# kvcache-ai/ktransformers

Hardware: NVIDIA H100
Metric: decode tok/s DeepSeek-V3 671B INT4 (Q4_K_M) MoE-block hot path; HBM GB/s vs roofline (higher is better)
Workload: dtype int8xint4/int6->int32 dp4a, fp32 scales+accumulate, bf16 in/out

## Files before the change

ktransformers_b200/csrc/gate.cuh:

```cuda
#pragma once
#include "common.cuh"

namespace ktb {

constexpr int kGateWarps = 4;
constexpr int kGateThreads = kGateWarps * 32;
constexpr int kGateTokTile = 8;

struct GateParams {
    const float* W;
    const void* x;
    int hidden_type, E, H, T, S;
    int top_k, n_group, topk_group, scoring, topk_method, norm_topk_prob;
    float routed_scaling_factor;
    const float* bias;
    float* partial;
    float* logits_out;
    int64_t* idx;
    float* w;
    const int* bsz;
    unsigned* ticket;
};

static inline int gate_splits(int E, int H, int nsms) {
    int S = nsms * 12 / E;
    if (S < 1) S = 1;
    if (S > 8) S = 8;
    while (S > 1 && H / 4 / S < 64) S--;
    return S;
}

constexpr int kGateEPT = 4;

static inline bool gate_config_ok(const ktb200_gate_config* c) {
    if (c->n_experts <= 0 || c->n_experts > kGateThreads * kGateEPT || c->hidden_size <= 0 || c->hidden_size % 4 || c->top_k <= 0 ||
        c->top_k > 32 || c->top_k > c->n_experts) {
        set_error("gate: bad shape (E=%d H=%d top_k=%d; E<=%d, top_k<=32, H%%4==0)", c->n_experts, c->hidden_size, c->top_k,
                  kGateThreads * kGateEPT);
        return false;
    }
    if (c->n_group < 1 || c->n_group > 32 || c->n_experts % c->n_group || c->topk_group < 1 || c->topk_group > c->n_group) {
        set_error("gate: bad grouping (n_group=%d topk_group=%d)", c->n_group, c->topk_group);
        return false;
    }
    if (c->scoring < 0 || c->scoring > 1 || c->topk_method < 0 || c->topk_method > 2) { set_error("gate: bad scoring/topk_method"); return false; }
    const int gs = c->n_experts / c->n_group;
    if (c->topk_method == 0 && c->n_group > 1 && gs < 2) {
        set_error("gate: noaux_tc needs at least 2 experts per group (E=%d n_group=%d)", c->n_experts, c->n_group);
        return false;
    }
    if (c->topk_method != 1 && c->n_group > 1 && c->top_k > c->topk_group * gs) {
        set_error("gate: top_k=%d exceeds the %d experts of topk_group=%d groups", c->top_k, c->topk_group * gs, c->topk_group);
        return false;
    }
    if (!is_hidden_type(c->hidden_type) || !c->weight) { set_error("gate: bad hidden_type or null weight"); return false; }
    return true;
}

__device__ __forceinline__ unsigned fkey(float f) {
    const unsigned u = __float_as_uint(f);
    return (u & 0x80000000u) ? ~u : (u | 0x80000000u);
}

__device__ __forceinline__ float fkey_inv(unsigned k) {
    return __uint_as_float((k & 0x80000000u) ? (k & 0x7fffffffu) : ~k);
}

template <int BAR>
__device__ __forceinline__ void gate_sync() {
    if (BAR == 0) __syncthreads();
    else asm volatile("bar.sync %0, %1;" ::"n"(BAR), "n"(kGateThreads) : "memory");
}
struct GateSel {
    int E, S, top_k, n_group, topk_group, scoring, topk_method, norm_topk_prob;
    float routed_scaling_factor;
    const float* bias;
    const float* partial;
};
template <int BAR>
__device__ void gate_select_token(const GateParams& pin, int t, float* sm, int64_t* idx_out, float* w_out, float* logits_out) {
    const GateSel p{pin.E, pin.S, pin.top_k, pin.n_group, pin.topk_group, pin.scoring, pin.topk_method, pin.norm_topk_prob,
                    pin.routed_scaling_factor, pin.bias, pin.partial};
    const int E = p.E, tid = threadIdx.x, lane = tid & 31, warp = tid >> 5;
    float* scores = sm;
    float* choice = sm + E;
    float* gsc = choice + E;
    unsigned* wbest = reinterpret_cast<unsigned*>(gsc + 32);
    float* red = reinterpret_cast<float*>(wbest + 2 * kGateWarps);

    float v[kGateEPT], pv[8][kGateEPT];
#pragma unroll
    for (int s = 0; s < 8; s++) {
        const float* pp = p.partial + ((long)t * p.S + s) * E;
#pragma unroll
        for (int i = 0; i < kGateEPT; i++) {
            const int e = tid + kGateThreads * i;
            pv[s][i] = (s < p.S && e < E) ? __ldcg(pp + e) : 0.f;
        }
    }
    float bv[kGateEPT];
#pragma unroll
    for (int i = 0; i < kGateEPT; i++) {
        const int e = tid + kGateThreads * i;
        bv[i] = (p.topk_method == 0 && p.bias && e < E) ? __ldg(p.bias + e) : 0.f;
    }
#pragma unroll
    for (int i = 0; i < kGateEPT; i++) {
        v[i] = 0.f;
#pragma unroll
        for (int s = 0; s < 8; s++)
            if (s < p.S) v[i] += pv[s][i];
    }
    if (logits_out) {
#pragma unroll
        for (int i = 0; i < kGateEPT; i++) {
            const int e = tid + kGateThreads * i;
            if (e < E) logits_out[(long)t * E + e] = v[i];
        }
    }
    if (p.scoring == 0) {
#pragma unroll
        for (int i = 0; i < kGateEPT; i++) v[i] = __fdiv_rn(1.0f, 1.0f + expf(-v[i]));
    } else {
        float m = -INFINITY;
#pragma unroll
        for (int i = 0; i < kGateEPT; i++) if (tid + kGateThreads * i < E) m = fmaxf(m, v[i]);
#pragma unroll
        for (int o = 16; o > 0; o >>= 1) m = fmaxf(m, __shfl_xor_sync(0xffffffffu, m, o));
        if (lane == 0) red[warp] = m;
        gate_sync<BAR>();
        m = red[0];
        for (int w = 1; w < kGateWarps; w++) m = fmaxf(m, red[w]);
        float sum = 0.f;
#pragma unroll
        for (int i = 0; i < kGateEPT; i++) {
            v[i] = (tid + kGateThreads * i < E) ? expf(v[i] - m) : 0.f;
            sum += v[i];
        }
        sum = warp_sum(sum);
        if (lane == 0) red[kGateWarps + warp] = sum;
        gate_sync<BAR>();
        sum = 0.f;
        for (int w = 0; w < kGateWarps; w++) sum += red[kGateWarps + w];
#pragma unroll
        for (int i = 0; i < kGateEPT; i++) v[i] = __fdiv_rn(v[i], sum);
    }
    float c[kGateEPT];
#pragma unroll
    for (int i = 0; i < kGateEPT; i++) {
        const int e = tid + kGateThreads * i;
        c[i] = -INFINITY;
        if (e < E) {
            c[i] = v[i] + bv[i];
            scores[e] = v[i];
            choice[e] = c[i];
        }
    }
    gate_sync<BAR>();

    if (p.n_group > 1 && p.topk_method != 1) {
        const int gs = E / p.n_group;
        for (int g = warp; g < p.n_group; g += kGateWarps) {
            float a1 = -INFINITY, a2 = -INFINITY;
            for (int i = lane; i < gs; i += 32) {
                const float x = choice[g * gs + i];
                if (x > a1) { a2 = a1; a1 = x; } else if (x > a2) { a2 = x; }
            }
            const unsigned k1 = fkey(a1);
            const unsigned mx1 = __reduce_max_sync(0xffffffffu, k1);
            const int wl = __ffs(__ballot_sync(0xffffffffu, k1 == mx1)) - 1;
            const unsigned mx2 = __reduce_max_sync(0xffffffffu, lane == wl ? fkey(a2) : k1);
            if (lane == 0) gsc[g] = (p.topk_method == 0) ? (fkey_inv(mx1) + fkey_inv(mx2)) : fkey_inv(mx1);
        }
        gate_sync<BAR>();
        const float fill = (p.topk_method == 0) ? -INFINITY : 0.0f;
#pragma unroll
        for (int i = 0; i < kGateEPT; i++) {
            const int e = tid + kGateThreads * i;
            if (e < E) {
                const int g = e / gs;
                const float mine = gsc[g];
                int rank = 0;
                for (int o = 0; o < p.n_group; o++) {
                    const float og = gsc[o];
                    rank += (og > mine || (og == mine && o < g)) ? 1 : 0;
                }
                if (rank >= p.topk_group) { c[i] = fill; choice[e] = fill; }
            }
        }
        gate_sync<BAR>();
    }

    if (warp == 0) {
        constexpr int EPL = kGateThreads * kGateEPT / 32;
        unsigned ck[EPL];
#pragma unroll
        for (int i = 0; i < EPL; i++) {
            const int e = lane + 32 * i;
            ck[i] = (e < E) ? fkey(choice[e]) : 0u;
        }
        float wsum = 0.f, myw = 0.f;
        long myidx = 0;
        for (int it = 0; it < p.top_k; it++) {
            unsigned bk = 0;
            int bi = 0x7fffffff;
#pragma unroll
            for (int i = 0; i < EPL; i++)
                if (ck[i] > bk) { bk = ck[i]; bi = lane + 32 * i; }
            const unsigned mx = __reduce_max_sync(0xffffffffu, bk);
            int win = __reduce_min_sync(0xffffffffu, (bk == mx) ? bi : 0x7fffffff);
            if (win == 0x7fffffff || win < 0 || win >= E) win = 0;
            const float wv = (p.topk_method == 2) ? choice[win] : scores[win];
#pragma unroll
            for (int i = 0; i < EPL; i++)
                if (lane + 32 * i == win) ck[i] = 0u;
            if (lane == it) { myw = wv; myidx = win; }
            wsum += wv;
        }
        if (lane < p.top_k) {
            float w = myw;
            const bool do_norm = p.top_k > 1 && p.norm_topk_prob;
            if (do_norm) w = __fdiv_rn(w, wsum + 1e-20f);
            if (p.topk_method == 0 || !do_norm) w = w * p.routed_scaling_factor;
            idx_out[lane] = myidx;
            w_out[lane] = w;
        }
    }
    gate_sync<BAR>();
}

template <int NT>
__device__ __forceinline__ void gate_dot(const GateParams& p, const float4* wrow, const float* xs, int nc4, int lane, int t0, int e,
                                         int s, int S, int nt = NT) {
    float acc[NT];
#pragma unroll
    for (int i = 0; i < NT; i++) acc[i] = 0.f;
    for (int cb = lane; cb < nc4; cb += 32 * 8) {
        float4 w[8];
#pragma unroll
        for (int u = 0; u < 8; u++) {
// ... 27 lines not shown
```

ktransformers_b200/csrc/moe_block.cu:

```cuda
#include <cstdlib>

#include "gate.cuh"
#include "gemv_bulk.cuh"
#include "handles.cuh"

namespace ktb {

constexpr int kBlockWarps = 15;
constexpr int kBlockWarpsLo = 12;

struct BlockParams {
    GateParams g;
    const void *w_gate, *w_up, *w_down;
    const void *s_gate, *s_up, *s_down;
    int n_local, id_offset;
    int H, I, k;
    int hidden_type, use_silu;
    float* inter;
    void* out;
    unsigned* sync;
    unsigned* ready;
    unsigned* status;
    uint8_t* stage_q;
    int16_t* stage_bs;
    float* stage_d;
    int nrows_max;
    int region_a;
    int ring_bytes;
    int prime_u, prime_d;
    unsigned long long* trace;
    const uint8_t* pf[3];
    unsigned pf_bytes[3];
};

__device__ __forceinline__ unsigned ld_acquire_u32(const unsigned* p) {
    unsigned v;
    asm volatile("ld.acquire.gpu.global.u32 %0, [%1];" : "=r"(v) : "l"(p) : "memory");
    return v;
}
__device__ __forceinline__ unsigned ld_acquire_sys_u32(const unsigned* p) {
    unsigned v;
    asm volatile("ld.acquire.sys.global.u32 %0, [%1];" : "=r"(v) : "l"(p) : "memory");
    return v;
}
__device__ __forceinline__ unsigned long long ep_now() {
    unsigned long long t;
    asm volatile("mov.u64 %0, %%globaltimer;" : "=l"(t));
    return t;
}
constexpr unsigned long long kEpTimeoutNs = 4000000000ull;
template <bool SYS>
__device__ __forceinline__ void wait_ge(const unsigned* p, unsigned target, unsigned* status) {
    unsigned long long t0 = 0;
    unsigned spins = 0;
    while ((int)((SYS ? ld_acquire_sys_u32(p) : ld_acquire_u32(p)) - target) < 0) {
        if ((++spins & 1023u) == 0) {
            const unsigned long long t = ep_now();
            if (!t0) t0 = t;
            else if (t - t0 > kEpTimeoutNs) { *status = 1; break; }
        }
    }
}

__device__ __forceinline__ void red_release_gpu_add(unsigned* p, unsigned v) {
    asm volatile("red.release.gpu.global.add.u32 [%0], %1;" ::"l"(p), "r"(v) : "memory");
}
__device__ __forceinline__ void grid_arrive(unsigned* counter, unsigned& gen) {
    __syncthreads();
    gen++;
    if (threadIdx.x == 0) red_release_gpu_add(counter, 1u);
}
__device__ __forceinline__ void grid_wait(unsigned* counter, unsigned gen) {
    if (threadIdx.x == 0) {
        const unsigned target = gen * gridDim.x;
        while (ld_acquire_u32(counter) < target) {}
    }
    __syncthreads();
}


__device__ __forceinline__ void trace_stamp(const BlockParams& p, int i) {
    if (p.trace) p.trace[blockIdx.x * 16 + i] = ep_now();
}
__device__ __forceinline__ void block_stamp(const BlockParams& p, int i) {
    if (threadIdx.x == 0) trace_stamp(p, i);
}

__device__ __forceinline__ float4 load_x4(const void* x, long i4, int type) {
    if (type == KTB200_TYPE_F32) return reinterpret_cast<const float4*>(x)[i4];
    const uint2 v = reinterpret_cast<const uint2*>(x)[i4];
    if (type == KTB200_TYPE_BF16)
        return make_float4(__uint_as_float(v.x << 16), __uint_as_float(v.x & 0xffff0000u), __uint_as_float(v.y << 16),
                           __uint_as_float(v.y & 0xffff0000u));
    const float2 a = __half22float2(*reinterpret_cast<const __half2*>(&v.x)), b = __half22float2(*reinterpret_cast<const __half2*>(&v.y));
    return make_float4(a.x, a.y, b.x, b.y);
}

struct BlockShared {
    BlockParams prm;
    int64_t ids[32];
    float w[32];
    int vs[36];
    int nv;
    unsigned skip;
    int ent_state[36];
    int last_cta;
};
constexpr int kBlockSharedBytes = (sizeof(BlockShared) + 15) & ~15;

struct BlockLay {
    uint8_t *xq, *aq;
    int16_t *xbs, *abs_;
    float *xdx, *adx, *sel, *partial;
    size_t ring_off;
};
template <int KBS>
__device__ __forceinline__ BlockLay block_layout(const BlockParams& p, uint8_t* smem) {
    const int nblk = p.H / QK_K, nb = p.I / QK_K, ns = p.k + (p.s_gate ? 1 : 0);
    uint8_t* a = smem + kBlockSharedBytes;
    BlockLay L;
    L.xq = a;
    L.xbs = reinterpret_cast<int16_t*>(a + (size_t)nblk * kActBlkStride);
    L.xdx = reinterpret_cast<float*>(a + (size_t)nblk * (kActBlkStride + 16));
    L.sel = reinterpret_cast<float*>(a + (((size_t)nblk * (kActBlkStride + 16 + 4) + 15) & ~(size_t)15));
    L.aq = a;
    L.abs_ = reinterpret_cast<int16_t*>(a + (size_t)ns * nb * kActBlkStride);
    L.adx = reinterpret_cast<float*>(a + (size_t)ns * nb * (kActBlkStride + 2 * KBS));
    L.partial = reinterpret_cast<float*>(a + p.region_a);
    L.ring_off = ((size_t)kBlockSharedBytes + p.region_a + (size_t)p.nrows_max * ns * 4 + 15) & ~(size_t)15;
    return L;
}

__device__ __forceinline__ void blk_quantize_x(int t) {
    extern __shared__ __align__(16) uint8_t smem[];
    const BlockParams& p = reinterpret_cast<const BlockShared*>(smem)->prm;
    const BlockLay L = block_layout<8>(p, smem);
    const int lane = threadIdx.x & 31, warp = threadIdx.x >> 5, W = blockDim.x >> 5, nblk = p.H / QK_K;
    float cur[8], nxt[8];
    int b = warp;
    if (b < nblk) load_block8(p.g.x, (long)t * p.H + (long)b * QK_K + lane * 8, p.hidden_type, cur);
#pragma unroll 1
    while (b < nblk) {
        const int bn = b + W;
        if (bn < nblk) load_block8(p.g.x, (long)t * p.H + (long)bn * QK_K + lane * 8, p.hidden_type, nxt);
        warp_quantize_q8k_block(cur, lane, reinterpret_cast<uint32_t*>(L.xq + (size_t)b * kActBlkStride), L.xdx + b, nullptr, L.xbs + b * 8);
#pragma unroll
        for (int i = 0; i < 8; i++) cur[i] = nxt[i];
        b = bn;
    }
}

__device__ __forceinline__ void blk_router(int t, bool& waited) {
    extern __shared__ __align__(16) uint8_t smem[];
    const BlockParams& p = reinterpret_cast<const BlockShared*>(smem)->prm;
    const int lane = threadIdx.x & 31, warp = threadIdx.x >> 5, W = blockDim.x >> 5;
    const int E = p.g.E, S = p.g.S, n4 = p.H / 4;
    const int gw = blockIdx.x * W + warp, tw = gridDim.x * W;
    for (int u = gw; u < E * S; u += tw) {
        const int s = u / E, e = u - s * E;
        const int c0 = (int)((long)n4 * s / S), nc4 = (int)((long)n4 * (s + 1) / S) - c0;
        const float4* wrow = reinterpret_cast<const float4*>(p.g.W + (long)e * p.H) + c0;
        const long xbase = (long)t * n4 + c0;
        float acc = 0.f;
        constexpr int NQ = 10;
        for (int cb = lane; cb < nc4; cb += 32 * NQ) {
            float4 w[NQ], xv[NQ];
#pragma unroll
            for (int q = 0; q < NQ; q++) {
                const int c = cb + 32 * q;
// ... 26 lines not shown
    extern __shared__ __align__(16) uint8_t smem[];
    const BlockParams& p = reinterpret_cast<const BlockShared*>(smem)->prm;
    const int lane = threadIdx.x & 31, warp = threadIdx.x >> 5, W = blockDim.x >> 5;
    const int E = p.g.E, S = p.g.S, n4 = p.H / 4, CH = p.ring_bytes / (16 * 32) * 32;
    const int gw = blockIdx.x * W + warp, tw = gridDim.x * W;
    const float4* ring = reinterpret_cast<const float4*>(smem + (ring_u32 - (uint32_t)__cvta_generic_to_shared(smem)));
    auto request = [&](int u, int cs) {
        const int s = u / E, e = u - s * E;
        const int c0 = (int)((long)n4 * s / S), nc4 = (int)((long)n4 * (s + 1) / S) - c0;
        if (lane == 0) {
            const uint32_t bytes = (uint32_t)min(CH, nc4 - cs) * 16u;
            mbar_expect_tx(bar, bytes);
            bulk_g2s(ring_u32, reinterpret_cast<const float4*>(p.g.W + (long)e * p.H) + c0 + cs, bytes, bar);
        }
    };
    if (gw < E * S) request(gw, 0);
    if (!waited) { griddep_wait(); waited = true; }
    blk_quantize_x(t);
    block_stamp(p, 1);
    for (int u = gw; u < E * S; u += tw) {
        const int s = u / E;
        const int c0 = (int)((long)n4 * s / S), nc4 = (int)((long)n4 * (s + 1) / S) - c0;
        const long xbase = (long)t * n4 + c0;
        float acc = 0.f;
        for (int cs = 0; cs < nc4; cs += CH) {
            if (u != gw || cs != 0) request(u, cs);
            const int n = min(CH, nc4 - cs);
            mbar_wait(bar, phase & 1u);
            phase ^= 1u;
            constexpr int NQ = 10;
            for (int cb = lane; cb < n; cb += 32 * NQ) {
                float4 xv[NQ];
#pragma unroll
                for (int q = 0; q < NQ; q++) {
                    const int c = cb + 32 * q;
                    if (c < n) xv[q] = load_x4(p.g.x, xbase + cs + c, p.hidden_type);
                }
#pragma unroll
                for (int q = 0; q < NQ; q++) {
                    const int c = cb + 32 * q;
                    if (c < n) {
                        const float4 w = ring[c];
                        acc = fmaf(w.x, xv[q].x, acc);
                        acc = fmaf(w.y, xv[q].y, acc);
                        acc = fmaf(w.z, xv[q].z, acc);
                        acc = fmaf(w.w, xv[q].w, acc);
                    }
                }
            }
            __syncwarp();
        }
        const float v = warp_sum(acc);
        if (lane == 0) p.g.partial[((long)t * S + s) * E + (u - s * E)] = v;
    }
}

__device__ __forceinline__ void blk_select(int t) {
    extern __shared__ __align__(16) uint8_t smem[];
    BlockShared& sh = *reinterpret_cast<BlockShared*>(smem);
    const BlockParams& p = sh.prm;
    const BlockLay L = block_layout<8>(p, smem);
    const int k = p.k;
    if ((threadIdx.x >> 5) < kGateWarps) {
        gate_select_token<1>(p.g, t, L.sel, sh.ids, sh.w, blockIdx.x == 0 ? p.g.logits_out : nullptr);
    }
    __syncthreads();
    block_stamp(p, 10);
    if (threadIdx.x < 32) {
        const int j = threadIdx.x, e0 = p.s_gate ? 1 : 0;
        const long e = j < k ? (long)sh.ids[j] - p.id_offset : -1;
        const bool own = e >= 0 && e < p.n_local;
        const unsigned m = __ballot_sync(0xffffffffu, own);
        if (own) sh.vs[e0 + __popc(m & ((1u << j) - 1u))] = j;
        if (j == 0) {
            sh.nv = e0 + __popc(m);
            sh.skip = ~m & ((1u << k) - 1u);
        }
    }
    if (blockIdx.x == 0 && threadIdx.x < k) {
        p.g.idx[(long)t * k + threadIdx.x] = sh.ids[threadIdx.x];
        p.g.w[(long)t * k + threadIdx.x] = sh.w[threadIdx.x];
    }
    __syncthreads();
}

__device__ __forceinline__ void entry_slice(int I, int ie, int& r0, int& len) {
    const unsigned s = (blockIdx.x + (unsigned)ie) % gridDim.x;
    r0 = (int)((unsigned long long)I * s / gridDim.x);
    len = (int)((unsigned long long)I * (s + 1) / gridDim.x) - r0;
}

constexpr unsigned kInterEmpty = 0xffffffffu;
__device__ __forceinline__ void st_relaxed_f32(float* p, float v) {
    asm volatile("st.relaxed.gpu.global.f32 [%0], %1;" ::"l"(p), "f"(v) : "memory");
}
__device__ __forceinline__ uint4 ld_relaxed_u4(const void* p) {
    uint4 v;
    asm volatile("ld.relaxed.gpu.global.v4.u32 {%0, %1, %2, %3}, [%4];" : "=r"(v.x), "=r"(v.y), "=r"(v.z), "=r"(v.w) : "l"(p) : "memory");
    return v;
}

template <int KBS>
__device__ __forceinline__ void quantise_block(const BlockParams& p, long gb, float* src) {
    const int lane = threadIdx.x & 31;
    uint4 v0, v1;
    unsigned long long t0 = 0;
    for (unsigned spins = 1;; spins++) {
        v0 = ld_relaxed_u4(src + lane * 8);
        v1 = ld_relaxed_u4(src + lane * 8 + 4);
        const bool here = v0.x != kInterEmpty && v0.y != kInterEmpty && v0.z != kInterEmpty && v0.w != kInterEmpty &&
                          v1.x != kInterEmpty && v1.y != kInterEmpty && v1.z != kInterEmpty && v1.w != kInterEmpty;
        if (__all_sync(0xffffffffu, here)) break;
        if ((spins & 255u) == 0) {
            const unsigned long long t = ep_now();
            if (!t0) t0 = t;
            else if (t - t0 > kEpTimeoutNs) { if (lane == 0) *p.status = 1; break; }
        }
    }
    const float x[8] = {__uint_as_float(v0.x), __uint_as_float(v0.y), __uint_as_float(v0.z), __uint_as_float(v0.w),
                        __uint_as_float(v1.x), __uint_as_float(v1.y), __uint_as_float(v1.z), __uint_as_float(v1.w)};
    warp_quantize_q8k_block(x, lane, reinterpret_cast<uint32_t*>(p.stage_q + gb * QK_K), p.stage_d + gb,
                            KBS == 16 ? p.stage_bs + gb * 16 : nullptr, KBS == 8 ? p.stage_bs + gb * 8 : nullptr);
    const uint4 empty = make_uint4(kInterEmpty, kInterEmpty, kInterEmpty, kInterEmpty);
    reinterpret_cast<uint4*>(src + lane * 8)[0] = empty;
    reinterpret_cast<uint4*>(src + lane * 8)[1] = empty;
    __syncwarp();
    if (lane == 0) {
        __threadfence();
        atomicExch(p.ready + gb, 2u);
    }
}

template <int KBS>
__device__ __forceinline__ void claim_entry(const BlockParams& p, int t, int slot) {
    const int lane = threadIdx.x & 31, ns = p.k + (p.s_gate ? 1 : 0), nb = p.I / QK_K;
    const long g0 = ((long)t * ns + slot) * nb;
    for (int c0 = 0; c0 < nb; c0 += 32) {
        const int nc = min(32, nb - c0), rot = (int)(blockIdx.x % nc);
        for (;;) {
            const unsigned fr = __ballot_sync(0xffffffffu, lane < nc && ld_acquire_u32(p.ready + g0 + c0 + lane) == 0u);
            if (!fr) break;
            const unsigned pref = fr & (~0u << rot);
            const int b = c0 + __ffs(pref ? pref : fr) - 1;
            unsigned won = 0;
            if (lane == 0) won = atomicCAS(p.ready + g0 + b, 0u, 1u) == 0u;
            if (__shfl_sync(0xffffffffu, won, 0)) quantise_block<KBS>(p, g0 + b, p.inter + ((long)t * ns + slot) * p.I + (long)b * QK_K);
        }
    }
}

template <int KBS>
__device__ __forceinline__ void entry_to_smem(BlockShared& sh, const BlockLay& L, int t, int ev, bool need) {
    const BlockParams& p = sh.prm;
    const int lane = threadIdx.x & 31;
    volatile int* state = &sh.ent_state[ev];
    int s = lane == 0 ? *state : 0;
    s = __shfl_sync(0xffffffffu, s, 0);
    if (s == 0) {
        if (lane == 0) s = atomicCAS(&sh.ent_state[ev], 0, 1) == 0 ? 3 : 1;
        s = __shfl_sync(0xffffffffu, s, 0);
    }
    if (s == 3) {
        const int nb = p.I / QK_K, slot = sh.vs[ev];
        const long g0 = ((long)t * (p.k + (p.s_gate ? 1 : 0)) + slot) * nb;
        for (int b = lane; b < nb; b += 32) wait_ge<false>(p.ready + g0 + b, 2u, p.status);
        __syncwarp();
// ... 45 lines not shown
    BlockShared& sh = *reinterpret_cast<BlockShared*>(smem);
    const int lane = threadIdx.x & 31, warp = threadIdx.x >> 5, W = blockDim.x >> 5;
    griddep_launch_dependents();
    bool waited = false;
    int Teff = p.g.T;
    if (p.g.bsz) { griddep_wait(); waited = true; Teff = min(Teff, *p.g.bsz); }
    const int k = p.k;
    const bool has_shared = p.s_gate != nullptr;
    uint32_t bar_u32, ring_u32;
    {
        const BlockLay L = block_layout<DownFmt::kBs>(p, smem);
        const int bar_bytes = (W * SU * 8 + 15) & ~15;
        bar_u32 = (uint32_t)__cvta_generic_to_shared(smem + L.ring_off) + warp * SU * 8;
        ring_u32 = (uint32_t)__cvta_generic_to_shared(smem + L.ring_off + bar_bytes) + warp * p.ring_bytes;
    }
    if (lane == 0) {
#pragma unroll
        for (int s = 0; s < SU; s++) mbar_init(bar_u32 + 8 * s, 1);
        mbar_fence_init();
        fence_proxy_async_smem();
    }
    {
        const uint32_t* src = reinterpret_cast<const uint32_t*>(&p);
        uint32_t* dst = reinterpret_cast<uint32_t*>(&sh.prm);
        for (int i = threadIdx.x; i < (int)(sizeof(BlockParams) / 4); i += blockDim.x) dst[i] = src[i];
    }
    if (threadIdx.x == 0 && has_shared) sh.vs[0] = k;
    uint32_t phase = 0;
    unsigned gen = 0;
    block_stamp(p, 0);

  for (int t = 0; t < Teff; t++) {
    __syncthreads();
    {
        const int nblk = p.H / QK_K, row_bytes = nblk * SZ_Q4_K;
        const int ns = k + (has_shared ? 1 : 0);
        int ie = 0, ir = 0, ir0 = 0, ilen = 0, ileft = 0, isub = 0;
        int ce = 0, cr = 0, cr0 = 0, clen = 0, cleft = 0, csub = 0;
        int stride = W, iend = 1;
        int slot_i = 0, slot_u = 0;
        auto advance = [&](int& e, int& r, int& r0, int& len, int n) {
            int off = r - r0 + n;
            while (off >= len && e + 1 < iend) { off -= len; e++; entry_slice(p.I, e, r0, len); }
            r = r0 + off;
        };
        auto start_list = [&](int e0, int e1, int first, int count, int stride_) {
            iend = e1;
            ie = e0;
            entry_slice(p.I, e0, ir0, ilen);
            ir = ir0;
            advance(ie, ir, ir0, ilen, first);
            ce = ie; cr = ir; cr0 = ir0; clen = ilen;
            ileft = cleft = count > 0 ? count : 0;
            stride = stride_;
        };
        auto issue_u = [&]() {
            if (ileft > 0 && isub - csub < SU) {
                if (lane == 0) {
                    const int s = sh.vs[ie];
                    const bool second = isub & 1;
                    const uint8_t* src;
                    if (s == k) {
                        src = reinterpret_cast<const uint8_t*>(second ? p.s_up : p.s_gate) + (long)ir * row_bytes;
                    } else {
                        const long e = (long)sh.ids[s] - p.id_offset;
                        src = reinterpret_cast<const uint8_t*>(second ? p.w_up : p.w_gate) + (e * p.I + ir) * row_bytes;
                    }
                    const uint32_t bar = bar_u32 + 8 * slot_i;
                    mbar_expect_tx(bar, (uint32_t)row_bytes);
                    bulk_g2s(ring_u32 + slot_i * row_bytes, src, (uint32_t)row_bytes, bar);
                }
                isub++;
                if (!(isub & 1)) {
                    ileft--;
                    advance(ie, ir, ir0, ilen, stride);
                }
                slot_i = (slot_i + 1 == SU) ? 0 : slot_i + 1;
            }
        };
        if (threadIdx.x < 36) sh.ent_state[threadIdx.x] = 0;
        blk_router_ring(t, waited, bar_u32, ring_u32, phase);
        block_stamp(p, 2);
        grid_arrive(p.sync, gen);
        if (has_shared && warp >= kGateWarps) {
            int r0, nr;
            entry_slice(p.I, 0, r0, nr);
            const int first = warp - kGateWarps, st = W - kGateWarps;
            start_list(0, 1, first, (nr - first + st - 1) / st, st);
        }
#pragma unroll
        for (int s = 0; s < SU; s++)
            if (s < p.prime_u) issue_u();
        grid_wait(p.sync, gen);
        block_stamp(p, 3);
        const BlockLay L = block_layout<DownFmt::kBs>(p, smem);
        const uint8_t* ring = smem + (ring_u32 - (uint32_t)__cvta_generic_to_shared(smem));
#pragma unroll 1
        for (int list = 0; list < 2; list++) {
            if (list == 1) {
                blk_select(t);
                block_stamp(p, 4);
                const int e0 = has_shared ? 1 : 0, nv = sh.nv;
                const unsigned G = gridDim.x, s0 = (blockIdx.x + (unsigned)e0) % G;
                auto rows_before = [&](unsigned sl) { return (int)(sl / G) * p.I + (int)((unsigned long long)p.I * (sl % G) / G); };
                const int total = rows_before(s0 + (unsigned)(nv - e0)) - rows_before(s0);
                start_list(e0, nv, warp, (total - warp + W - 1) / W, W);
#pragma unroll
                for (int s = 0; s < SU; s++) issue_u();
            }
            float acc_first = 0.f;
            bool stamp_first = list == 1 && warp == 0;
            while (cleft > 0) {
                mbar_wait(bar_u32 + 8 * slot_u, (phase >> slot_u) & 1u);
                phase ^= 1u << slot_u;
                if (stamp_first) {
                    if (lane == 0) trace_stamp(p, 11);
                    stamp_first = false;
                }
                const uint8_t* row0 = ring + slot_u * row_bytes;
                float acc = 0.f;
                if (lane < nblk)
                    acc = q4k_block_dot(row0 + lane * SZ_Q4_K, L.xq + (size_t)lane * kActBlkStride,
                                        *reinterpret_cast<const uint4*>(L.xbs + lane * 8), L.xdx[lane]);
                __syncwarp();
                slot_u = (slot_u + 1 == SU) ? 0 : slot_u + 1;
                csub++;
                issue_u();
                if (csub & 1) { acc_first = acc; continue; }
                float g = acc_first, uu = acc;
#pragma unroll
                for (int o = 16; o > 0; o >>= 1) {
                    g += __shfl_xor_sync(0xffffffffu, g, o);
                    uu += __shfl_xor_sync(0xffffffffu, uu, o);
                }
                if (lane == 0) st_relaxed_f32(p.inter + ((long)t * ns + sh.vs[ce]) * p.I + cr, (p.use_silu ? act_silu(g) : act_relu(g)) * uu);
                cleft--;
                advance(ce, cr, cr0, clen, stride);
            }
        }
        __syncthreads();
        block_stamp(p, 5);
    }
    {
        const int nb = p.I / QK_K, nrb = RW * nb, item_bytes = nrb * DownFmt::kBlockBytes;
        const int quads = p.H / RW;
        const int q0 = (int)((long)quads * blockIdx.x / gridDim.x), nquads = (int)((long)quads * (blockIdx.x + 1) / gridDim.x) - q0;
        const int nv = sh.nv;
        const int Wd = W - 1;
        int ni = warp < Wd ? nquads * nv - warp : 0;
        ni = ni > 0 ? (ni + Wd - 1) / Wd : 0;
        int dvi = 0, dq = 0, dss = 0, dcons = 0;
        if (ni > 0) { dvi = warp / nquads; dq = warp - dvi * nquads; }
        int evi = dvi, eq = dq;
        int dslot_i = 0, dslot_u = 0;
        auto issue_d = [&]() {
            if (dss < ni && dss - dcons < SD) {
                if (lane == 0) {
                    const int j = sh.vs[dvi];
                    long row = (long)(q0 + dq) * RW;
                    const uint8_t* wbase = reinterpret_cast<const uint8_t*>(p.w_down);
                    if (j == k) wbase = reinterpret_cast<const uint8_t*>(p.s_down);
                    else row += ((long)sh.ids[j] - p.id_offset) * p.H;
                    const uint32_t bar = bar_u32 + 8 * dslot_i;
                    mbar_expect_tx(bar, (uint32_t)item_bytes);
                    bulk_g2s(ring_u32 + dslot_i * item_bytes, wbase + (row >> 2) * item_bytes, (uint32_t)item_bytes, bar);
                }
                dss++;
                dq += Wd;
                while (dq >= nquads) { dq -= nquads; dvi++; }
                dslot_i = (dslot_i + 1 == SD) ? 0 : dslot_i + 1;
            }
        };
#pragma unroll
        for (int s = 0; s < SD; s++) issue_d();
        const BlockLay L = block_layout<DownFmt::kBs>(p, smem);
        if (warp == W - 1) {
            for (int ev = 0; ev < nv; ev++) claim_entry<DownFmt::kBs>(p, t, sh.vs[ev]);
        }
        if (t == Teff - 1 && warp == W - 1) {
#pragma unroll
            for (int r = 0; r < 3; r++) {
                if (p.pf[r]) {
                    const unsigned per = ((p.pf_bytes[r] / gridDim.x) + 15u) & ~15u;
                    const unsigned lo = per * blockIdx.x, hi = min(p.pf_bytes[r], lo + per);
                    for (unsigned o = lo + lane * 4096u; o < hi; o += 32u * 4096u) prefetch_l2_bulk(p.pf[r] + o, min(4096u, hi - o) & ~15u);
                }
            }
        }

        const uint8_t* ring = smem + (ring_u32 - (uint32_t)__cvta_generic_to_shared(smem));
        const int ns = k + (has_shared ? 1 : 0);
        for (int n = 0; n < ni; n++) {
            if (eq < Wd) {
                entry_to_smem<DownFmt::kBs>(sh, L, t, evi, true);
                if (evi + 1 < nv) entry_to_smem<DownFmt::kBs>(sh, L, t, evi + 1, false);
            }
            mbar_wait(bar_u32 + 8 * dslot_u, (phase >> dslot_u) & 1u);
            phase ^= 1u << dslot_u;
            const uint8_t* sl = ring + dslot_u * item_bytes;
            const int j = sh.vs[evi];
            float res;
            {
                float acc[RW] = {0.f, 0.f, 0.f, 0.f};
                for (int f = lane; f < nrb; f += 32) {
                    const int rw = f / nb, blk = f - rw * nb;
                    const int ab = j * nb + blk;
                    const float val = DownFmt::dot(sl, f, nrb, L.aq + (size_t)ab * kActBlkStride, L.abs_ + ab * DownFmt::kBs, L.adx[ab]);
                    acc[0] += rw == 0 ? val : 0.f; acc[1] += rw == 1 ? val : 0.f; acc[2] += rw == 2 ? val : 0.f; acc[3] += rw == 3 ? val : 0.f;
                }
                res = warp_reduce4(acc[0], acc[1], acc[2], acc[3], lane);
            }
            __syncwarp();
            dslot_u = (dslot_u + 1 == SD) ? 0 : dslot_u + 1;
            dcons++;
            issue_d();
            if ((lane & 7) == 0) L.partial[(eq * RW + (lane >> 3)) * ns + j] = res;
            eq += Wd;
            while (eq >= nquads) { eq -= nquads; evi++; }
        }
        __syncthreads();
        block_stamp(p, 8);
        blk_combine<DownFmt::kBs>(t);
        block_stamp(p, 9);
    }
  }

    __syncthreads();
    if (threadIdx.x == 0) sh.last_cta = atomicAdd(p.sync + 1, 1u) == gridDim.x - 1;
    __syncthreads();
    if (sh.last_cta) {
        const int nready = Teff * (k + (has_shared ? 1 : 0)) * (p.I / QK_K);
        for (int i = threadIdx.x; i < nready; i += blockDim.x) p.ready[i] = 0;
        if (threadIdx.x == 0) {
            p.sync[0] = 0;
            p.sync[1] = 0;
        }
        __threadfence();
    }
}


constexpr int kEpWorldMax = 8;
constexpr int kEpPairsMax = 64;

struct EpExtra {
    int rank, world, phase_mask, pa;
    int msg_bytes;
    int inter_shared_row;
    float* shared_out;
    uint8_t* msg[kEpWorldMax];
    float* part[kEpWorldMax];
    unsigned* flags[kEpWorldMax];
    int ep_off;
};
struct EpParams { BlockParams b; EpExtra x; };

struct EpShared {
    EpExtra x;
    unsigned epoch;
    int np;
    int pair_src[kEpPairsMax];
    int pair_e[kEpPairsMax];
    float pair_w[kEpPairsMax];
    int tok_slot[2];
};

__device__ __forceinline__ void st_release_sys_u32(unsigned* p, unsigned v) {
    asm volatile("st.release.sys.global.u32 [%0], %1;" ::"l"(p), "r"(v) : "memory");
}
__device__ __forceinline__ void red_release_sys_add(unsigned* p, unsigned v) {
    asm volatile("red.release.sys.global.add.u32 [%0], %1;" ::"l"(p), "r"(v) : "memory");
}

template <int KBS>
__device__ __forceinline__ void ep_quantize_row(const BlockParams& p, const uint8_t* row, uint8_t* slot_base) {
    const int lane = threadIdx.x & 31, warp = threadIdx.x >> 5, W = blockDim.x >> 5, nblk = p.H / QK_K;
    uint8_t* xq = slot_base;
    int16_t* xbs = reinterpret_cast<int16_t*>(slot_base + (size_t)nblk * kActBlkStride);
    float* xdx = reinterpret_cast<float*>(slot_base + (size_t)nblk * (kActBlkStride + 2 * KBS));
    for (int b = warp; b < nblk; b += W) {
        float x[8];
        const long e0 = (long)b * QK_K + lane * 8;
        if (p.hidden_type == KTB200_TYPE_F32) {
            const float4 a = __ldcg(reinterpret_cast<const float4*>(row) + e0 / 4), c = __ldcg(reinterpret_cast<const float4*>(row) + e0 / 4 + 1);
            x[0] = a.x; x[1] = a.y; x[2] = a.z; x[3] = a.w; x[4] = c.x; x[5] = c.y; x[6] = c.z; x[7] = c.w;
        } else {
            const uint4 raw = __ldcg(reinterpret_cast<const uint4*>(row) + e0 / 8);
            const uint32_t w[4] = {raw.x, raw.y, raw.z, raw.w};
#pragma unroll
            for (int i = 0; i < 4; i++) {
                if (p.hidden_type == KTB200_TYPE_BF16) {
                    x[2 * i] = __uint_as_float(w[i] << 16);
                    x[2 * i + 1] = __uint_as_float(w[i] & 0xffff0000u);
                } else {
                    const float2 f = __half22float2(*reinterpret_cast<const __half2*>(&w[i]));
                    x[2 * i] = f.x; x[2 * i + 1] = f.y;
                }
            }
        }
        warp_quantize_q8k_block(x, lane, reinterpret_cast<uint32_t*>(xq + (size_t)b * kActBlkStride), xdx + b,
                                KBS == 16 ? xbs + b * 16 : nullptr, KBS == 8 ? xbs + b * 8 : nullptr);
    }
}

template <class DownFmt>
__global__ void __launch_bounds__(kBlockWarpsLo * 32, 1) moe_ep_block_kernel(const EpParams pp) {
    constexpr int RW = 4, SU = 4, SD = 2;
    extern __shared__ __align__(16) uint8_t smem[];
    BlockShared& sh = *reinterpret_cast<BlockShared*>(smem);
    EpShared& es = *reinterpret_cast<EpShared*>(smem + pp.x.ep_off);
    const BlockParams& p = pp.b;
    const int lane = threadIdx.x & 31, warp = threadIdx.x >> 5, W = blockDim.x >> 5;
    griddep_launch_dependents();
    bool waited = false;
    const int k = p.k, world = pp.x.world, rank = pp.x.rank, mask = pp.x.phase_mask;
    const bool has_shared = p.s_gate != nullptr;
    const int nblk = p.H / QK_K, row_bytes = nblk * SZ_Q4_K;
    const int nb = p.I / QK_K;
    uint32_t bar_u32, ring_u32;
    {
// ... 605 lines not shown
static int env_fused() {
    static int v = [] { const char* e = getenv("KTB200_FUSED"); return e ? atoi(e) : 1; }();
    return v;
}

}

using namespace ktb;

extern "C" int ktb200_moe_block_forward(const ktb200_gate_config* gc, ktb200_moe* m, ktb200_mlp* sh, int qlen, const void* input,
                                        void* output, int64_t* idx, float* w, const int* bsz, void* stream) {
    if (!gc || !m || !input || !output || !idx || !w) { set_error("null pointer"); return KTB200_EINVAL; }
    if (!gate_config_ok(gc)) return KTB200_EINVAL;
    if (!m->loaded) { set_error("Not Loaded"); return KTB200_ESTATE; }
    if (sh && !sh->loaded) { set_error("shared expert: Not Loaded"); return KTB200_ESTATE; }
    if (qlen <= 0) return KTB200_OK;
    const ktb200_moe_config& c = m->cfg;
    const int k = gc->top_k;
    if (gc->hidden_size != c.hidden_size || gc->hidden_type != c.hidden_type) { set_error("moe_block: gate and experts disagree on the hidden size / type"); return KTB200_EINVAL; }
    if (k <= 0 || k > c.routed_expert_num) { set_error("moe_block: top_k=%d outside (0, routed_expert_num=%d]", k, c.routed_expert_num); return KTB200_EINVAL; }
    if (qlen > c.group_max_len) { set_error("forward: qlen=%d exceeds group_max_len=%d", qlen, c.group_max_len); return KTB200_EINVAL; }

    const FmtId fd = pick_fmt(c.down_type, m->down_layout);
    const bool sh_ok = !sh || (sh->H == c.hidden_size && sh->I == c.intermediate_size && sh->hidden_type == c.hidden_type &&
                               sh->gate_type == c.gate_type && sh->up_type == c.up_type && sh->down_type == c.down_type &&
                               sh->gu_soa == m->gu_soa && sh->down_layout == m->down_layout && c.use_silu);
    const int nblk = c.hidden_size / QK_K, nb = c.intermediate_size / QK_K;
    bool fused = env_fused() && qlen <= kBlockMaxTokens && sh_ok && c.gate_type == KTB200_TYPE_Q4_K && c.up_type == KTB200_TYPE_Q4_K &&
                 (fd == FMT_Q6K4T || fd == FMT_Q4K) && nblk >= 16 && nblk <= 32 && c.hidden_size % 4 == 0 && k <= 31;
    DeviceGuard guard(m->device);
    const int dev = m->device;
    cudaStream_t s = (cudaStream_t)stream;
    BlockParams p{};
    size_t smem = 0;
    int W = 0, G = 0;
    if (fused) {
        const int ns = k + (sh ? 1 : 0);
        const int kbs = fd == FMT_Q6K4T ? 16 : 8, bbytes = fd == FMT_Q6K4T ? SZ_Q6_K : SZ_Q4_K;
        const size_t item = (size_t)4 * nb * bbytes, row = (size_t)nblk * SZ_Q4_K;
        G = num_sms(dev);
        if (G > c.intermediate_size) G = c.intermediate_size;
        if (G > c.hidden_size / 4) G = c.hidden_size / 4;
        const int quads = c.hidden_size / 4;
        p.nrows_max = ((quads + G - 1) / G) * 4;
        const size_t xq = (((size_t)nblk * (kActBlkStride + 16 + 4) + 15) & ~(size_t)15) + ((size_t)2 * gc->n_experts + 32 + 4 * kGateWarps) * 4;
        const size_t aqb = (size_t)ns * nb * (kActBlkStride + 2 * kbs + 4);
        p.region_a = (int)(((xq > aqb ? xq : aqb) + 15) & ~(size_t)15);
        size_t base = (size_t)kBlockSharedBytes + p.region_a + (size_t)p.nrows_max * ns * 4;
        base = (base + 15) & ~(size_t)15;
        static const int want_w = [] { const char* e = getenv("KTB200_BLK_WARPS"); return e ? atoi(e) : kBlockWarpsLo; }();
        const int su = want_w > kBlockWarpsLo ? 3 : 4;
        size_t ring = su * row > 2 * item ? su * row : 2 * item;
        p.ring_bytes = (int)ring;
        W = base + 64 < 232448 - 1024 ? (int)((232448 - 1024 - base - 16) / (ring + 8 * su)) : 0;
        if (W > (want_w > kBlockWarpsLo ? kBlockWarps : kBlockWarpsLo)) W = want_w > kBlockWarpsLo ? kBlockWarps : kBlockWarpsLo;
        if (want_w >= 8 && W > want_w) W = want_w;
        if (want_w > kBlockWarpsLo && W <= kBlockWarpsLo) W = 0;
        smem = base + (((size_t)W * su * 8 + 15) & ~(size_t)15) + (size_t)W * ring;
        if (W < 8 || c.hidden_size % 4 || item % 16 || c.intermediate_size < 1) fused = false;
    }
    if (!fused) {
        int rc = ktb200_moe_gate_forward(gc, qlen, input, idx, w, nullptr, bsz, stream);
        if (rc) return rc;
        return ktb200_moe_forward_shared(m, sh, qlen, k, idx, w, input, output, bsz, stream);
    }

    const int S = gate_splits(gc->n_experts, gc->hidden_size, num_sms(dev));
    p.g = GateParams{gc->weight, input, gc->hidden_type, gc->n_experts, gc->hidden_size, qlen, S, k, gc->n_group, gc->topk_group,
                     gc->scoring, gc->topk_method, gc->norm_topk_prob, gc->routed_scaling_factor, gc->bias, m->blk_partial, nullptr,
                     idx, w, bsz, nullptr};
    p.w_gate = c.gate_proj; p.w_up = c.up_proj; p.w_down = c.down_proj;
    p.s_gate = sh ? sh->gate : nullptr; p.s_up = sh ? sh->up : nullptr; p.s_down = sh ? sh->down : nullptr;
    p.n_local = c.expert_num; p.id_offset = c.expert_id_offset;
    p.H = c.hidden_size; p.I = c.intermediate_size; p.k = k; p.hidden_type = c.hidden_type; p.use_silu = c.use_silu;
    const unsigned flip = m->blk_flip++ & 1u;
    p.inter = m->blk_inter; p.out = output; p.sync = m->blk_sync + 2 * flip; p.trace = g_btrace;
    p.status = m->blk_sync + kBlkStatusWord;
    p.ready = m->blk_sync + kBlkReadyWord + flip * blk_ready_words(c);
    p.stage_q = m->blk_stage;
    p.stage_bs = reinterpret_cast<int16_t*>(m->blk_stage + blk_ready_words(c) * (size_t)QK_K);
    p.stage_d = reinterpret_cast<float*>(m->blk_stage + blk_ready_words(c) * (size_t)(QK_K + 32));
    for (int r = 0; r < 3; r++) { p.pf[r] = (const uint8_t*)m->pf[r]; p.pf_bytes[r] = (unsigned)m->pf_bytes[r]; }
    static const int prime_u = [] { const char* e = getenv("KTB200_BLK_PRIME_U"); return e ? atoi(e) : 3; }();
    p.prime_u = prime_u;

    void* args[] = {&p};
    const void* fn;
    if (W > kBlockWarpsLo) fn = fd == FMT_Q6K4T ? (const void*)moe_block_kernel<BulkQ6K4T, kBlockWarps> : (const void*)moe_block_kernel<BulkQ4K, kBlockWarps>;
    else fn = fd == FMT_Q6K4T ? (const void*)moe_block_kernel<BulkQ6K4T, kBlockWarpsLo> : (const void*)moe_block_kernel<BulkQ4K, kBlockWarpsLo>;
    static const int coop = [] { const char* e = getenv("KTB200_BLK_COOP"); return e ? atoi(e) : 1; }();
    static const int pdl = [] { const char* e = getenv("KTB200_BLK_PDL"); return e ? atoi(e) : 1; }();
    auto separate = [&]() -> int {
        int rc = ktb200_moe_gate_forward(gc, qlen, input, idx, w, nullptr, bsz, stream);
        if (rc) return rc;
        return ktb200_moe_forward_shared(m, sh, qlen, k, idx, w, input, output, bsz, stream);
    };
    {
        static size_t limit[4][64] = {};
        static int resident[4][64] = {};
        const int v = (W > kBlockWarpsLo ? 2 : 0) + (fd == FMT_Q6K4T ? 1 : 0);
        if (limit[v][dev & 63] < smem) {
            KTB_CUDA_CHECK(cudaFuncSetAttribute(fn, cudaFuncAttributeMaxDynamicSharedMemorySize, (int)smem));
            int per_sm = 0;
            KTB_CUDA_CHECK(cudaOccupancyMaxActiveBlocksPerMultiprocessor(&per_sm, fn, W * 32, smem));
            resident[v][dev & 63] = per_sm * num_sms(dev);
            limit[v][dev & 63] = smem;
        }
        if (resident[v][dev & 63] < G) return separate();
    }
    cudaLaunchConfig_t lc{};
    lc.gridDim = dim3(G); lc.blockDim = dim3(W * 32); lc.dynamicSmemBytes = smem; lc.stream = s;
    cudaLaunchAttribute at[2];
    int na = 0;
    if (coop) { at[na].id = cudaLaunchAttributeCooperative; at[na].val.cooperative = 1; na++; }
    if (pdl) { at[na].id = cudaLaunchAttributeProgrammaticStreamSerialization; at[na].val.programmaticStreamSerializationAllowed = 1; na++; }
    lc.attrs = at; lc.numAttrs = na;
    cudaError_t le = cudaLaunchKernelExC(&lc, fn, args);
    if (le != cudaSuccess && coop && pdl && (le == cudaErrorNotSupported || le == cudaErrorInvalidValue)) {
        (void)cudaGetLastError();
        lc.numAttrs = 1;
        le = cudaLaunchKernelExC(&lc, fn, args);
    }
    if (le == cudaErrorCooperativeLaunchTooLarge) {
        (void)cudaGetLastError();
        return separate();
    }
    if (le != cudaSuccess) { set_error("moe_block launch failed: %s", cudaGetErrorString(le)); return KTB200_ECUDA; }
    count_launch(1);
    return KTB200_OK;
}

extern "C" long ktb200_ep_msg_bytes(int hidden_size, int hidden_type) { return (long)hidden_size * type_size(hidden_type) + 128; }

namespace ktb {
static int ep_block_params(EpParams& pp, const ktb200_gate_config* gc, ktb200_moe* m, ktb200_mlp* sh, const ktb200_ep_comm* comm,
                           const void* x_own, void* y_out, int64_t* idx, float* w, int phase_mask) {
    const ktb200_moe_config& c = m->cfg;
    const int k = gc->top_k, world = comm->world;
    BlockParams& p = pp.b;
    const int S = gate_splits(gc->n_experts, gc->hidden_size, num_sms(m->device));
    p.g = GateParams{gc->weight, x_own, gc->hidden_type, gc->n_experts, gc->hidden_size, 1, S, k, gc->n_group, gc->topk_group,
                     gc->scoring, gc->topk_method, gc->norm_topk_prob, gc->routed_scaling_factor, gc->bias, m->blk_partial, nullptr,
                     idx, w, nullptr, nullptr};
    p.w_gate = c.gate_proj; p.w_up = c.up_proj; p.w_down = c.down_proj;
    p.s_gate = sh ? sh->gate : nullptr; p.s_up = sh ? sh->up : nullptr; p.s_down = sh ? sh->down : nullptr;
    p.n_local = c.expert_num; p.id_offset = c.expert_id_offset;
    p.H = c.hidden_size; p.I = c.intermediate_size; p.k = k; p.hidden_type = c.hidden_type; p.use_silu = c.use_silu;
    p.inter = m->inter; p.out = y_out; p.sync = m->blk_sync + 2 * (m->blk_flip++ & 1u); p.trace = g_btrace;
    p.prime_u = 3; p.prime_d = 2;
    pp.x.rank = comm->rank; pp.x.world = world; pp.x.phase_mask = phase_mask;
    pp.x.msg_bytes = (int)ktb200_ep_msg_bytes(c.hidden_size, c.hidden_type);
    pp.x.inter_shared_row = world * k;
    pp.x.shared_out = m->blk_partial + 16384;
    for (int r = 0; r < world; r++) {
        if (!comm->token_bufs[r] || !comm->partial_bufs[r] || !comm->flag_bufs[r]) { set_error("ep_block: null peer pointer for rank %d", r); return KTB200_EINVAL; }
        pp.x.msg[r] = (uint8_t*)comm->token_bufs[r]; pp.x.part[r] = comm->partial_bufs[r]; pp.x.flags[r] = comm->flag_bufs[r];
    }
    return KTB200_OK;
}

static int ep_block_resident(const void* fn, int variant, int G, int W, size_t smem, int dev) {
    static size_t limit[10][64] = {};
    static int resident[10][64] = {};
    if (limit[variant][dev & 63] < smem) {
        KTB_CUDA_CHECK(cudaFuncSetAttribute(fn, cudaFuncAttributeMaxDynamicSharedMemorySize, (int)smem));
        int per_sm = 0;
        KTB_CUDA_CHECK(cudaOccupancyMaxActiveBlocksPerMultiprocessor(&per_sm, fn, W * 32, smem));
// ... 231 lines not shown
```

profiles/block_trace.py:

```python
#!/usr/bin/env python
import argparse
import ctypes as C
import os
import sys

sys.path.insert(0, os.path.dirname(os.path.dirname(os.path.abspath(__file__))))
ap = argparse.ArgumentParser()
ap.add_argument("--graph", action="store_true", help="58 launches in one CUDA graph with PDL, as bench.py times them")
args = ap.parse_args()
if args.graph:
    os.environ["KTB200_BLK_COOP"] = "0"
import numpy as np
import torch

from ktransformers_b200 import native
from ktransformers_b200.util.synth import synth_blocks

lib = native.lib()
E, K, H, I = 256, 8, 7168, 2048
Q4_K, Q6_K, BF16 = 12, 14, 30
N_LAYERS = 58
S = lambda: torch.cuda.current_stream().cuda_stream
layers = []
for l in range(4 if args.graph else 3):
    g, u, d = synth_blocks(Q4_K, E * I * H, device="cuda", seed=3 * l), synth_blocks(Q4_K, E * I * H, device="cuda", seed=3 * l + 1), synth_blocks(Q6_K, E * H * I, device="cuda", seed=3 * l + 2)
    sg, su, sd = synth_blocks(Q4_K, I * H, device="cuda", seed=100 + l), synth_blocks(Q4_K, I * H, device="cuda", seed=200 + l), synth_blocks(Q6_K, H * I, device="cuda", seed=300 + l)
    cfg = native.MoeConfig(E, K, H, I, 64, 10, 8, 1, g.data_ptr(), u.data_ptr(), d.data_ptr(), Q4_K, Q4_K, Q6_K, BF16, 0)
    moe = C.c_void_p(); native.check(lib.ktb200_moe_create(C.byref(cfg), 0, C.byref(moe))); native.check(lib.ktb200_moe_load_weights(moe, S()))
    mlp = C.c_void_p(); native.check(lib.ktb200_mlp_create(H, I, sg.data_ptr(), su.data_ptr(), sd.data_ptr(), Q4_K, Q4_K, Q6_K, BF16, 8, 0, C.byref(mlp)))
    native.check(lib.ktb200_mlp_load_weights(mlp, S()))
    W = torch.randn(E, H, device="cuda"); b = (0.01 if args.graph else 1.0) * torch.randn(E, device="cuda")
    gc = native.GateConfig(E, H, K, 8, 4, 0, 0, 1, 2.5, W.data_ptr(), b.data_ptr(), BF16)
    layers.append((gc, moe, mlp, (g, u, d, sg, su, sd, W, b)))
x = (torch.randn(1, H, device="cuda") / 100).to(torch.bfloat16)
n_sm = torch.cuda.get_device_properties(torch.cuda.current_device()).multi_processor_count
names = ["start", "x quantised (under barrier 1)", "router partials written", "grid barrier 1 passed", "top-k selected",
         "gate/up done (CTA)", "entry 0 ready (its a in smem)", "last entry ready (its a in smem)", "down tiles done (CTA)", "combined + stored",
         "  (top-k done, before the work-list build)", "first routed gate/up row landed (warp 0)"]
NS = len(names)
PRELUDE = [0, 2, 1, 3, 10, 4, 11]


def table(t, title):
    print(f"{'boundary':46s} {'first':>8s} {'median':>8s} {'last':>8s}   ({title})")
    for i in sorted(range(NS), key=lambda i: np.median(t[:, i])):
        print(f"{names[i]:46s} {t[:, i].min():8.2f} {np.median(t[:, i]):8.2f} {t[:, i].max():8.2f}")


if not args.graph:
    y = torch.zeros(1, H, dtype=torch.bfloat16, device="cuda")
    ids = torch.zeros(1, K, dtype=torch.int64, device="cuda"); wts = torch.zeros(1, K, device="cuda")
    trace = torch.zeros(n_sm * 16, dtype=torch.int64, device="cuda")
    acc = []
    for rep in range(12):
        gc, moe, mlp, _ = layers[rep % 3]
        lib.ktb200_debug_block_trace(trace.data_ptr())
        native.check(lib.ktb200_moe_block_forward(C.byref(gc), moe, mlp, 1, x.data_ptr(), y.data_ptr(), ids.data_ptr(), wts.data_ptr(), None, S()))
        torch.cuda.synchronize()
        t = trace.cpu().numpy().reshape(n_sm, 16)[:, :NS].astype(np.float64)
        t -= t[:, 0].min()
        if rep >= 3:
            acc.append(t)
    lib.ktb200_debug_block_trace(None)
    table(np.mean(acc, axis=0) / 1e3, f"us after the first CTA started; mean of {len(acc)} eager launches")
    sys.exit(0)

y = torch.zeros(N_LAYERS, 1, H, dtype=torch.bfloat16, device="cuda")
ids = torch.zeros(N_LAYERS, 1, K, dtype=torch.int64, device="cuda"); wts = torch.zeros(N_LAYERS, 1, K, device="cuda")
trace = torch.zeros(N_LAYERS, n_sm, 16, dtype=torch.int64, device="cuda")


def step(traced):
    for l in range(N_LAYERS):
        gc, moe, mlp, _ = layers[l % 4]
        lib.ktb200_debug_block_trace(trace[l].data_ptr() if traced else None)
        native.check(lib.ktb200_moe_block_forward(C.byref(gc), moe, mlp, 1, x.data_ptr(), y[l].data_ptr(), ids[l].data_ptr(), wts[l].data_ptr(), None, S()))
    lib.ktb200_debug_block_trace(None)


step(False)
torch.cuda.synchronize()
side = torch.cuda.Stream()
side.wait_stream(torch.cuda.current_stream())
with torch.cuda.stream(side):
    step(True)
torch.cuda.current_stream().wait_stream(side)
torch.cuda.synchronize()
gr = torch.cuda.CUDAGraph()
with torch.cuda.graph(gr):
    step(True)
for _ in range(5):
    gr.replay()
torch.cuda.synchronize()
trace.zero_()
e0, e1 = torch.cuda.Event(enable_timing=True), torch.cuda.Event(enable_timing=True)
e0.record(); gr.replay(); e1.record()
torch.cuda.synchronize()
ms = e0.elapsed_time(e1)
tr = trace.cpu().numpy()[:, :, :NS].astype(np.float64)
print(f"# {torch.cuda.get_device_name()}: one replay of {N_LAYERS} launches in {ms:.3f} ms = {1e3 * ms / N_LAYERS:.1f} us per launch (stamps on)")
rel_start = np.mean([tr[l] - tr[l, :, 0].min() for l in range(1, N_LAYERS)], axis=0) / 1e3
table(rel_start, f"us after this launch's first CTA started; mean of launches 1..{N_LAYERS - 1} of one replay")
print()
rel_prev = np.mean([tr[l] - tr[l - 1, :, 9].max() for l in range(1, N_LAYERS)], axis=0) / 1e3
table(rel_prev, f"us after the previous launch's last CTA stored its output; mean of launches 1..{N_LAYERS - 1}")
print()
per = np.array([tr[l, :, 9].max() - tr[l - 1, :, 9].max() for l in range(1, N_LAYERS)]) / 1e3
print(f"last-CTA-done to last-CTA-done per launch: median {np.median(per):.2f} us, min {per.min():.2f}, max {per.max():.2f}")
print("prelude split (median CTA, us after the previous launch's last CTA):")
for i in PRELUDE:
    print(f"  {names[i].strip():46s} {np.median(rel_prev[:, i]):8.2f}")
```

Measured before the change: 165.5.

## Split top-k selection onto gate warps with named barriers, overlap shared-expert work

Top-k selection now runs only in the four gate warps using a named-barrier handshake. The other warps finish their shared-expert slice and prime the routed gate/up prefetch after the gate warps signal their inputs are read, then wait on a second named barrier for the ids. This replaces a full-CTA selection and __syncthreads so that selection overlaps with the shared-expert GEMV. It also drops a trailing __threadfence and forces prime_u to be at least 1. The named-barrier IDs and thread counts add risk of deadlock or races if arrive/sync counts mismatch.

New measurement: 169.3 (median of 6 runs). 2.3% higher.

```diff
diff --git a/ktransformers_b200/csrc/gate.cuh b/ktransformers_b200/csrc/gate.cuh
--- a/ktransformers_b200/csrc/gate.cuh
+++ b/ktransformers_b200/csrc/gate.cuh
@@ -77,7 +77,7 @@
     const float* bias;
     const float* partial;
 };
-template <int BAR>
+template <int BAR, int ARRIVE = 0>
 __device__ void gate_select_token(const GateParams& pin, int t, float* sm, int64_t* idx_out, float* w_out, float* logits_out) {
     const GateSel p{pin.E, pin.S, pin.top_k, pin.n_group, pin.topk_group, pin.scoring, pin.topk_method, pin.norm_topk_prob,
                     pin.routed_scaling_factor, pin.bias, pin.partial};
@@ -156,6 +156,7 @@
             choice[e] = c[i];
         }
     }
+    if (ARRIVE) asm volatile("bar.arrive %0, %1;" ::"n"(ARRIVE), "r"(blockDim.x) : "memory");
     gate_sync<BAR>();
 
     if (p.n_group > 1 && p.topk_method != 1) {
diff --git a/ktransformers_b200/csrc/moe_block.cu b/ktransformers_b200/csrc/moe_block.cu
--- a/ktransformers_b200/csrc/moe_block.cu
+++ b/ktransformers_b200/csrc/moe_block.cu
@@ -85,6 +85,9 @@
 __device__ __forceinline__ void block_stamp(const BlockParams& p, int i) {
     if (threadIdx.x == 0) trace_stamp(p, i);
 }
+__device__ __forceinline__ void trace_latest(const BlockParams& p, int i) {
+    if (p.trace) atomicMax(p.trace + blockIdx.x * 16 + i, ep_now());
+}
 
 __device__ __forceinline__ float4 load_x4(const void* x, long i4, int type) {
     if (type == KTB200_TYPE_F32) return reinterpret_cast<const float4*>(x)[i4];
@@ -277,6 +280,37 @@
         p.g.w[(long)t * k + threadIdx.x] = sh.w[threadIdx.x];
     }
     __syncthreads();
+}
+
+constexpr int kBarTopkIn = 2, kBarIds = 3;
+__device__ __forceinline__ void named_bar_sync(int id, int n) { asm volatile("bar.sync %0, %1;" ::"r"(id), "r"(n) : "memory"); }
+__device__ __forceinline__ void named_bar_arrive(int id, int n) { asm volatile("bar.arrive %0, %1;" ::"r"(id), "r"(n) : "memory"); }
+
+__device__ __forceinline__ void blk_select_fused(int t) {
+    extern __shared__ __align__(16) uint8_t smem[];
+    BlockShared& sh = *reinterpret_cast<BlockShared*>(smem);
+    const BlockParams& p = sh.prm;
+    const BlockLay L = block_layout<8>(p, smem);
+    const int k = p.k;
+    gate_select_token<1, kBarTopkIn>(p.g, t, L.sel, sh.ids, sh.w, blockIdx.x == 0 ? p.g.logits_out : nullptr);
+    block_stamp(p, 12);
+    if (threadIdx.x < 32) {
+        const int j = threadIdx.x, e0 = p.s_gate ? 1 : 0;
+        const long e = j < k ? (long)sh.ids[j] - p.id_offset : -1;
+        const bool own = e >= 0 && e < p.n_local;
+        const unsigned m = __ballot_sync(0xffffffffu, own);
+        if (own) sh.vs[e0 + __popc(m & ((1u << j) - 1u))] = j;
+        if (j == 0) {
+            sh.nv = e0 + __popc(m);
+            sh.skip = ~m & ((1u << k) - 1u);
+        }
+    }
+    if (blockIdx.x == 0 && threadIdx.x < k) {
+        p.g.idx[(long)t * k + threadIdx.x] = sh.ids[threadIdx.x];
+        p.g.w[(long)t * k + threadIdx.x] = sh.w[threadIdx.x];
+    }
+    named_bar_sync(1, kGateThreads);
+    named_bar_arrive(kBarIds, blockDim.x);
 }
 
 __device__ __forceinline__ void entry_slice(int I, int ie, int& r0, int& len) {
@@ -488,23 +522,33 @@
         blk_router_ring(t, waited, bar_u32, ring_u32, phase);
         block_stamp(p, 2);
         grid_arrive(p.sync, gen);
+        block_stamp(p, 14);
         if (has_shared && warp >= kGateWarps) {
             int r0, nr;
             entry_slice(p.I, 0, r0, nr);
             const int first = warp - kGateWarps, st = W - kGateWarps;
             start_list(0, 1, first, (nr - first + st - 1) / st, st);
         }
-#pragma unroll
-        for (int s = 0; s < SU; s++)
-            if (s < p.prime_u) issue_u();
         grid_wait(p.sync, gen);
         block_stamp(p, 3);
+        if (warp >= kGateWarps) {
+            named_bar_sync(kBarTopkIn, blockDim.x);
+#pragma unroll
+            for (int s = 0; s < SU; s++)
+                if (s < p.prime_u) issue_u();
+        }
         const BlockLay L = block_layout<DownFmt::kBs>(p, smem);
         const uint8_t* ring = smem + (ring_u32 - (uint32_t)__cvta_generic_to_shared(smem));
 #pragma unroll 1
         for (int list = 0; list < 2; list++) {
             if (list == 1) {
-                blk_select(t);
+                if (warp < kGateWarps) {
+                    blk_select_fused(t);
+                } else {
+                    if (lane == 0) trace_latest(p, 13);
+                    named_bar_sync(kBarIds, blockDim.x);
+                    if (warp == kGateWarps && lane == 0) trace_stamp(p, 10);
+                }
                 block_stamp(p, 4);
                 const int e0 = has_shared ? 1 : 0, nv = sh.nv;
                 const unsigned G = gridDim.x, s0 = (blockIdx.x + (unsigned)e0) % G;
@@ -641,7 +685,6 @@
             p.sync[0] = 0;
             p.sync[1] = 0;
         }
-        __threadfence();
     }
 }
 
@@ -1413,7 +1456,7 @@
     p.stage_d = reinterpret_cast<float*>(m->blk_stage + blk_ready_words(c) * (size_t)(QK_K + 32));
     for (int r = 0; r < 3; r++) { p.pf[r] = (const uint8_t*)m->pf[r]; p.pf_bytes[r] = (unsigned)m->pf_bytes[r]; }
     static const int prime_u = [] { const char* e = getenv("KTB200_BLK_PRIME_U"); return e ? atoi(e) : 3; }();
-    p.prime_u = prime_u;
+    p.prime_u = prime_u > 0 ? prime_u : 1;
 
     void* args[] = {&p};
     const void* fn;
diff --git a/profiles/block_trace.py b/profiles/block_trace.py
--- a/profiles/block_trace.py
+++ b/profiles/block_trace.py
@@ -36,9 +36,10 @@
 n_sm = torch.cuda.get_device_properties(torch.cuda.current_device()).multi_processor_count
 names = ["start", "x quantised (under barrier 1)", "router partials written", "grid barrier 1 passed", "top-k selected",
          "gate/up done (CTA)", "entry 0 ready (its a in smem)", "last entry ready (its a in smem)", "down tiles done (CTA)", "combined + stored",
-         "  (top-k done, before the work-list build)", "first routed gate/up row landed (warp 0)"]
+         "  (selection barrier passed: every warp starts the routed rows)", "first routed gate/up row landed (warp 0)",
+         "  (top-k done in warps 0..3: the ids are there)", "  (warps 4.. done with the shared expert's slice)", "  (CTA arrived: every warp's router units done)"]
 NS = len(names)
-PRELUDE = [0, 2, 1, 3, 10, 4, 11]
+PRELUDE = [0, 1, 2, 14, 3, 12, 13, 10, 4, 11]
 
 
 def table(t, title):
```
